# nubcico/EAV

Measured on AMD Instinct MI355X. Metric: EEGNet training samples/sec (fwd+CE+bwd+Adam), whole job, higher is better.
Workload: dtype f32; 1 GPU; EEGNet_tor(5, Chans=30, Samples=10000, kernLength=300, F1=8, D=8, F2=64) train step on x[64,1,30,10000] fp32 per GPU (BASELINE.json configs[1]); global_batch=64, per_gpu_batch=64, parallelism=dp1

## Files before the change

### eav_amd/_lib.py

```python
from __future__ import annotations

import ctypes as C
import os

_HERE = os.path.dirname(os.path.abspath(__file__))
LIB_PATH = os.environ.get("EAV_LIB_PATH") or os.path.join(_HERE, "libeav_hip.so")


class EavError(RuntimeError):
    pass


_p = C.c_void_p
_i = C.c_int
_i64 = C.c_int64
_u64 = C.c_uint64
_f = C.c_float
_d = C.c_double

SIGNATURES = {
    "eav_reduce_partials": [_p, _i, _i64, _i, _f, _p, _p],
    "eav_bn_finalize": [_p, _i, _i, _d, _p, _p, _p, _p, _i, _f, _f, _p, _p, _p, _p, _p],
    "eav_bn_bwd_finalize": [_p, _i, _i, _d, _i, _p, _p, _p, _p, _p],
    "eav_reduce_and_bn_bwd_finalize": [_p, _i, _i64, _i, _p, _p, _i, _i, _d, _i, _p, _p, _p, _p, _p, _i, _i, _d, _i, _p, _p, _p,
                                       _p, _p],
    "eav_renorm_rows": [_p, _i, _i, _f, _p],
    "eav_renorm_rows2": [_p, _i, _i, _p, _i, _i, _f, _p],
    "eav_eegnet_step_prologue": [_p, _p, _p, _p, _p, _p, _p, _p],
    "eav_eegnet_fir_fwd": [_p, _p, _p, _p, _i, _i, _i, _i, _p],
    "eav_eegnet_fir_wgrad": [_p, _p, _p, _p, _p, _i, _i, _i, _i, _p],
    "eav_eegnet_fir_fwd_indexed": [_p, _p, _p, _p, _p, _i, _i, _i, _i, _p],
    "eav_eegnet_fir_fwd_fft": [_p, _p, _p, _p, _p, _i, _i, _i, _i, _p],
    "eav_eegnet_fir_wgrad_fft": [_p, _p, _p, _p, _p, _p, _p, _i, _i, _i, _i, _p],
    "eav_eegnet_fir_wgrad_indexed": [_p, _p, _p, _p, _p, _p, _i, _i, _i, _i, _p],
    "eav_eegnet_dw_fwd": [_p, _p, _p, _p, _p, _i, _i, _i, _p],
    "eav_eegnet_dw_fwd_pool_eval": [_p, _p, _p, _p, _p, _p, _p, _i, _i, _i, _p],
    "eav_eegnet_dw_bwd": [_p, _p, _p, _p, _p, _p, _p, _i, _i, _i, _p],
    "eav_eegnet_dw_bwd_fused": [_p, _p, _p, _p, _p, _p, _p, _p, _p, _i, _i, _i, _f, _u64, _p, _p, _p],
    "eav_eegnet_dw_bwd_fused_eval": [_p, _p, _p, _p, _p, _p, _p, _p, _p, _p, _i, _i, _i, _f, _u64, _p, _p, _p],
    "eav_bn_elu_pool_fwd": [_p, _p, _p, _i, _i, _i, _i, _f, _u64, _p, _p, _p],
    "eav_bn_elu_pool_bwd_reduce": [_p, _p, _p, _p, _i, _i, _i, _i, _f, _u64, _p, _p, _p],
    "eav_bn_elu_pool_bwd_apply": [_p, _p, _p, _p, _p, _i, _i, _i, _i, _f, _u64, _p, _p, _p],
    "eav_bn_elu_pool_bwd_eval": [_p, _p, _p, _p, _p, _i, _i, _i, _i, _f, _u64, _p, _p, _p],
    "eav_conv64_prep_weights": [_p, _p, _p, _p],
    "eav_conv64_fwd": [_p, _p, _p, _p, _i, _i, _i, _p],
    "eav_conv64_wgrad": [_p, _p, _p, _i, _i, _i, _p],
    "eav_conv64_fft_fwd": [_p, _p, _p, _p, _p, _i, _i, _i, _p],
    "eav_conv64_fft_wgrad": [_p, _p, _p, _i, _i, _p],
    "eav_conv64_fft_bwd": [_p, _p, _p, _p, _p, _f, _u64, _p, _p, _p, _p, _p, _i, _i, _p],
    "eav_dense_softmax_fwd": [_p, _p, _p, _p, _p, _i, _i, _i, _p],
    "eav_dense_softmax_bwd": [_p, _p, _p, _p, _p, _p, _p, _i, _i, _i, _p],
    "eav_ce_fwd_bwd": [_p, _p, _p, _p, _p, _p, _i, _i, _p],
    "eav_dense_wide_fwd": [_p, _p, _p, _p, _i, _i, _i, _p],
    "eav_dense_wide_bwd": [_p, _p, _p, _p, _p, _p, _p, _i, _i, _i, _p],
    "eav_ce_wide_fwd_bwd": [_p, _p, _p, _p, _p, _p, _p, _i, _i, _p],
    "eav_bce_logits_fwd_bwd": [_p, _p, _p, _p, _p, _p, _i, _i, _p],
    "eav_mse_fwd_bwd": [_p, _p, _p, _p, _p, _i, _i, _p],
    "eav_scale_by_scalar": [_p, _p, _i64, _p],
    "eav_adam_step": [_p, _p, _p, _p, _i64, _f, _f, _f, _f, _f, _i64, _i, _p, _p],
    "eav_adam_step_scaled": [_p, _p, _p, _p, _i64, _f, _f, _f, _f, _f, _i64, _i, _p, _p, _p],
    "eav_grad_sumsq": [_p, _i, _i64, _p, _p],
    "eav_grad_fold": [_p, _p, _i, _i64, _p, _i, _p, _p],
    "eav_grad_clip_finish": [_p, _i64, _f, _p, _p],
    "eav_scale_ranges": [_p, _i, _i64, _p, _p],
    "eav_counter_inc": [_p, _p],
    "eav_counter_inc4": [_p, _p, _p, _p, _p],
# ... 245 lines not shown
```

### eav_amd/csrc/eav_common.hip

```cpp
#include "eav_common.h"

#include <stdarg.h>
#include <stdio.h>

#include "../../include/eav_hip.h"

static thread_local char g_err[512] = "";

int eav_set_error(int code, const char* fmt, ...) {
  va_list ap;
  va_start(ap, fmt);
  vsnprintf(g_err, sizeof(g_err), fmt, ap);
  va_end(ap);
  return code;
}

extern "C" const char* eav_last_error(void) { return g_err; }
extern "C" int eav_abi_version(void) { return EAV_ABI_VERSION; }

__global__ __launch_bounds__(256) void reduce_partials_kernel(const float* __restrict__ part, int nparts,
                                                              int64_t stride, int n, float scale,
                                                              float* __restrict__ out) {
  __shared__ double sh[16][17];
  const int ol = threadIdx.x & 15, pl = threadIdx.x >> 4;
// ... 129 lines not shown

extern "C" int eav_bn_finalize(const float* part, int nparts, int nch, double count, const float* gamma,
                               const float* beta, float* running_mean, float* running_var, int training,
                               float momentum, float eps, float* mean, float* invstd, float* scale, float* shift,
                               void* stream) {
  EAV_REQUIRE(nch > 0 && gamma && beta && running_mean && running_var && mean && invstd && scale && shift,
              "eav_bn_finalize: bad arguments");
  EAV_REQUIRE(!training || (part && nparts > 0 && count > 0), "eav_bn_finalize: training needs partials");
  hipLaunchKernelGGL(bn_finalize_kernel, dim3(nch), dim3(256), 0, (hipStream_t)stream, part, nparts, nch,
                     count, gamma, beta, running_mean, running_var, training, momentum, eps, mean, invstd, scale,
                     shift);
  EAV_CHECK_LAUNCH("eav_bn_finalize");
  return EAV_OK;
}

__device__ __forceinline__ void bn_bwd_finalize_body(const float* __restrict__ part, int nparts, int nch, double count,
                                                     int training, float* __restrict__ dgamma, float* __restrict__ dbeta,
                                                     float* __restrict__ m1, float* __restrict__ m2, int c) {
  __shared__ double shs[256], shq[256];
  double s = 0.0, q = 0.0;
  for (int p = threadIdx.x; p < nparts; p += 256) {
    s += (double)part[(int64_t)p * 2 * nch + c];
    q += (double)part[(int64_t)p * 2 * nch + nch + c];
  }
  shs[threadIdx.x] = s;
  shq[threadIdx.x] = q;
  __syncthreads();
  for (int o = 128; o > 0; o >>= 1) {
    if (threadIdx.x < o) {
      shs[threadIdx.x] += shs[threadIdx.x + o];
      shq[threadIdx.x] += shq[threadIdx.x + o];
    }
    __syncthreads();
  }
  if (threadIdx.x != 0) return;
  s = shs[0];
  q = shq[0];
  dbeta[c] = (float)s;
  dgamma[c] = (float)q;
  m1[c] = training ? (float)(s / count) : 0.f;
  m2[c] = training ? (float)(q / count) : 0.f;
}

__global__ void bn_bwd_finalize_kernel(const float* __restrict__ part, int nparts, int nch, double count,
                                       int training, float* __restrict__ dgamma, float* __restrict__ dbeta,
                                       float* __restrict__ m1, float* __restrict__ m2) {
  bn_bwd_finalize_body(part, nparts, nch, count, training, dgamma, dbeta, m1, m2, blockIdx.x);
}

struct BnBwdJob {
  const float* part;
  int nparts, nch, training;
  double count;
  float *dgamma, *dbeta, *m1, *m2;
};

// ... 36 lines not shown
                     n / 4, 1.f, out, nred, a, b);
  EAV_CHECK_LAUNCH("eav_reduce_and_bn_bwd_finalize");
  return EAV_OK;
}

extern "C" int eav_bn_bwd_finalize(const float* part, int nparts, int nch, double count, int training,
                                   float* dgamma, float* dbeta, float* m1, float* m2, void* stream) {
  EAV_REQUIRE(part && nparts > 0 && nch > 0 && count > 0 && dgamma && dbeta && m1 && m2,
              "eav_bn_bwd_finalize: bad arguments");
  hipLaunchKernelGGL(bn_bwd_finalize_kernel, dim3(nch), dim3(256), 0, (hipStream_t)stream, part, nparts,
                     nch, count, training, dgamma, dbeta, m1, m2);
  EAV_CHECK_LAUNCH("eav_bn_bwd_finalize");
  return EAV_OK;
}

__global__ void renorm_rows_kernel(float* __restrict__ w, int rows, int cols, float maxnorm, float* __restrict__ w_b,
                                   int cols_b) {
  __shared__ float red[8];
  int r = blockIdx.x;
  if (r >= rows) {
    r -= rows;
    w = w_b;
    cols = cols_b;
  }
  float* row = w + (int64_t)r * cols;
  const bool vec = (cols & 3) == 0 && (reinterpret_cast<uintptr_t>(row) & 15) == 0;
  float v[1] = {0.f};
  if (vec) {
    const float4* row4 = reinterpret_cast<const float4*>(row);
    const int n4 = cols >> 2;
// ... 54 lines not shown
```

### eav_amd/csrc/eegnet_block.hip

```cpp
#include "eav_common.h"
#include "../../include/eav_hip.h"

namespace {

constexpr int F1 = 8, DD = 8, CHMAX = 32;

__device__ __forceinline__ void ld4s(const float* p, int i, int n, bool vec, float (&v)[4]) {
  if (vec && i + 3 < n) {
    const f32x4 a = __builtin_nontemporal_load(reinterpret_cast<const f32x4*>(p + i));
    v[0] = a[0]; v[1] = a[1]; v[2] = a[2]; v[3] = a[3];
  } else {
#pragma unroll
    for (int e = 0; e < 4; ++e) v[e] = (i + e < n) ? p[i + e] : 0.f;
  }
}
__device__ __forceinline__ void st4s(float* p, int i, int n, bool vec, const float (&v)[4]) {
  if (vec && i + 3 < n) {
    __builtin_nontemporal_store((f32x4){v[0], v[1], v[2], v[3]}, reinterpret_cast<f32x4*>(p + i));
  } else {
#pragma unroll
    for (int e = 0; e < 4; ++e)
      if (i + e < n) p[i + e] = v[e];
  }
}
// ... 96 lines not shown
      float ps = 0.f;
#pragma unroll
      for (int e = 0; e < 4; ++e) ps += elu_f(sc2 * acc[d][e] + sh2);
      p2[((int64_t)b * CH + ch) * (S / 4) + t / 4] = ps * 0.25f;
    }
  }
  block_sum_nt<NT, 16>(st, red);
  if (threadIdx.x < 16) {
    const int nch = F1 * DD;
    float* dst = part + ((int64_t)b * gridDim.x + chunk) * 2 * nch;
    const int d = threadIdx.x & 7;
    dst[(threadIdx.x < 8 ? 0 : nch) + f * DD + d] = st[0];
  }
}

template <int P>
__global__ __launch_bounds__(256) void pool_fwd_kernel(const float* __restrict__ in, const float* __restrict__ bn,
                                                       float* __restrict__ out, int CH, int T, float drop_p,
                                                       uint64_t seed_in,
    const uint8_t* __restrict__ mask, const uint64_t* __restrict__ seed_dev) {
  const uint64_t seed = dropout_seed(seed_in, seed_dev);
  const int row = blockIdx.x, ch = row % CH;
  const float sc = bn[2 * CH + ch], sh = bn[3 * CH + ch];
  const int To = T / P;
  const float* src = in + (int64_t)row * T;
  const bool vec = (T & 3) == 0;
  for (int to = threadIdx.x; to < To; to += 256) {
    float s = 0.f;
#pragma unroll
    for (int j = 0; j < P; j += 4) {
      float v[4];
      ld4(src, to * P + j, T, vec, v);
#pragma unroll
      for (int e = 0; e < 4; ++e) s += elu_f(sc * v[e] + sh);
    }
    const uint64_t oi = (uint64_t)row * To + to;
    out[oi] = s * (1.0f / P) * dropout_mult_row(drop_p, seed, mask, oi, (uint64_t)row);
  }
}

template <int P>
__global__ __launch_bounds__(256) void pool_bwd_reduce_kernel(const float* __restrict__ dp,
                                                              const float* __restrict__ u,
                                                              const float* __restrict__ bn, float* __restrict__ part,
                                                              int CH, int T, float drop_p, uint64_t seed_in,
    const uint8_t* __restrict__ mask, const uint64_t* __restrict__ seed_dev) {
  const uint64_t seed = dropout_seed(seed_in, seed_dev);
  __shared__ float red[8];
  const int row = blockIdx.x, ch = row % CH, b = row / CH;
  const float mean = bn[ch], invstd = bn[CH + ch], sc = bn[2 * CH + ch], sh = bn[3 * CH + ch];
  const int To = T / P;
  const float* src = u + (int64_t)row * T;
// ... 311 lines not shown
                                       int B, int C, int S, float drop_p, uint64_t seed, const uint8_t* mask,
                                       const uint64_t* seed_dev, void* stream) {
  return dw_bwd_fused_launch("eav_eegnet_dw_bwd_fused", y1, z, dp2, bn2, bn1, w2, g1, stat_part, w_part, nullptr, B, C, S,
                             drop_p, seed, mask, seed_dev, stream);
}

extern "C" int eav_eegnet_dw_bwd_fused_eval(const float* y1, const float* z, const float* dp2, const float* bn2,
                                            const float* bn1, const float* w2, float* g1, float* stat_part, float* w_part,
                                            float* bn2_part, int B, int C, int S, float drop_p, uint64_t seed,
                                            const uint8_t* mask, const uint64_t* seed_dev, void* stream) {
  EAV_REQUIRE(bn2_part, "eav_eegnet_dw_bwd_fused_eval: bad arguments");
  return dw_bwd_fused_launch("eav_eegnet_dw_bwd_fused_eval", y1, z, dp2, bn2, bn1, w2, g1, stat_part, w_part, bn2_part, B, C,
                             S, drop_p, seed, mask, seed_dev, stream);
}

extern "C" int eav_bn_elu_pool_fwd(const float* in, const float* bn, float* out, int B, int CH, int T, int P,
                                   float drop_p, uint64_t seed, const uint8_t* mask, const uint64_t* seed_dev, void* stream) {
  EAV_REQUIRE(in && bn && out && B > 0 && CH > 0 && T >= P, "eav_bn_elu_pool_fwd: bad arguments");
  EAV_REQUIRE(P == 4 || P == 8, "eav_bn_elu_pool_fwd: pool %d not in {4,8}", P);
  EAV_REQUIRE(drop_p > -1.f && drop_p < 1.f, "eav_bn_elu_pool_fwd: dropout %f outside (-1,1)", drop_p);
  if (P == 4)
    hipLaunchKernelGGL(pool_fwd_kernel<4>, dim3(B * CH), dim3(256), 0, (hipStream_t)stream, in, bn, out, CH, T,
                       drop_p, seed, mask, seed_dev);
  else
    hipLaunchKernelGGL(pool_fwd_kernel<8>, dim3(B * CH), dim3(256), 0, (hipStream_t)stream, in, bn, out, CH, T,
                       drop_p, seed, mask, seed_dev);
  EAV_CHECK_LAUNCH("eav_bn_elu_pool_fwd");
  return EAV_OK;
}

extern "C" int eav_bn_elu_pool_bwd_reduce(const float* dp, const float* u, const float* bn, float* part, int B,
                                          int CH, int T, int P, float drop_p, uint64_t seed, const uint8_t* mask,
                                          const uint64_t* seed_dev, void* stream) {
  EAV_REQUIRE(dp && u && bn && part && B > 0 && CH > 0 && T >= P, "eav_bn_elu_pool_bwd_reduce: bad arguments");
  EAV_REQUIRE(P == 4 || P == 8, "eav_bn_elu_pool_bwd_reduce: pool %d not in {4,8}", P);
  if (P == 4)
    hipLaunchKernelGGL(pool_bwd_reduce_kernel<4>, dim3(B * CH), dim3(256), 0, (hipStream_t)stream, dp, u, bn, part,
                       CH, T, drop_p, seed, mask, seed_dev);
  else
    hipLaunchKernelGGL(pool_bwd_reduce_kernel<8>, dim3(B * CH), dim3(256), 0, (hipStream_t)stream, dp, u, bn, part,
                       CH, T, drop_p, seed, mask, seed_dev);
  EAV_CHECK_LAUNCH("eav_bn_elu_pool_bwd_reduce");
  return EAV_OK;
// ... 33 lines not shown
```

### eav_amd/csrc/head_optim.hip

```cpp
#include "eav_common.h"
#include "../../include/eav_hip.h"

namespace {

constexpr int NCMAX = 16;

__global__ __launch_bounds__(1024) void dense_softmax_fwd_kernel(const float* __restrict__ in,
                                                                 const float* __restrict__ w,
                                                                 const float* __restrict__ bias,
                                                                 float* __restrict__ logits, float* __restrict__ probs,
                                                                 int NF, int NC) {
  __shared__ float red[16 * NCMAX];
  const int b = blockIdx.x;
  const int lane = threadIdx.x & 63, wave = threadIdx.x >> 6;
  const float* src = in + (int64_t)b * NF;
  float acc[NCMAX];
#pragma unroll
  for (int j = 0; j < NCMAX; ++j) acc[j] = 0.f;
  if ((NF & 3) == 0) {
    const int nq = NF >> 2;
    if (NC <= 5) {
      for (int i0 = threadIdx.x; i0 < nq; i0 += 4096) {
        float4 v[4], wv[4][5];
#pragma unroll
// ... 45 lines not shown
    lg[threadIdx.x] = s + bias[threadIdx.x];
  }
  __syncthreads();
  if (threadIdx.x == 0) {
    float mx = lg[0];
    for (int j = 1; j < NC; ++j) mx = fmaxf(mx, lg[j]);
    float e[NCMAX], s = 0.f;
    for (int j = 0; j < NC; ++j) { e[j] = expf(lg[j] - mx); s += e[j]; }
    for (int j = 0; j < NC; ++j) {
      if (logits) logits[b * NC + j] = lg[j];
      if (probs) probs[b * NC + j] = e[j] / s;
    }
  }
}

__global__ __launch_bounds__(256) void dense_softmax_bwd_kernel(const float* __restrict__ dout,
                                                                const float* __restrict__ probs,
                                                                const float* __restrict__ in,
                                                                const float* __restrict__ w, float* __restrict__ dw,
                                                                float* __restrict__ dbias, float* __restrict__ din,
                                                                int B, int NF, int NC) {
  extern __shared__ float dl[];
  float* pw = dl + B * NC;
  for (int idx = threadIdx.x; idx < B * NC; idx += blockDim.x) {
    const int b = idx / NC;
    float v = dout[idx];
    if (probs) {
      float dot = 0.f;
      for (int j = 0; j < NC; ++j) dot += dout[b * NC + j] * probs[b * NC + j];
      v = probs[idx] * (v - dot);
    }
    dl[idx] = v;
  }
  __syncthreads();
  if (blockIdx.x == 0 && threadIdx.x < NC) {
    float s = 0.f;
    for (int b = 0; b < B; ++b) s += dl[b * NC + threadIdx.x];
    dbias[threadIdx.x] = s;
  }
  const int f = threadIdx.x & 63, slice = threadIdx.x >> 6;
  const int i = blockIdx.x * 64 + f;
  const bool live = i < NF;
  float wv[NCMAX], acc[NCMAX];
#pragma unroll
  for (int j = 0; j < NCMAX; ++j) {
    wv[j] = (live && j < NC) ? w[(int64_t)j * NF + i] : 0.f;
    acc[j] = 0.f;
  }
  for (int b0 = slice; b0 < B; b0 += 32) {
    float v[8];
#pragma unroll
    for (int u = 0; u < 8; ++u) v[u] = (live && b0 + 4 * u < B) ? in[(int64_t)(b0 + 4 * u) * NF + i] : 0.f;
#pragma unroll
    for (int u = 0; u < 8; ++u) {
      const int b = b0 + 4 * u;
      if (b < B) {
        float d = 0.f;
#pragma unroll
        for (int j = 0; j < NCMAX; ++j)
          if (j < NC) {
            const float g = dl[b * NC + j];
            acc[j] += g * v[u];
            d += wv[j] * g;
          }
        if (din && live) din[(int64_t)b * NF + i] = d;
      }
    }
  }
#pragma unroll
  for (int j = 0; j < NCMAX; ++j) pw[(slice * NCMAX + j) * 64 + f] = acc[j];
  __syncthreads();
  if (slice == 0 && live) {
#pragma unroll
    for (int j = 0; j < NCMAX; ++j)
      if (j < NC)
        dw[(int64_t)j * NF + i] = (pw[j * 64 + f] + pw[(NCMAX + j) * 64 + f]) + (pw[(2 * NCMAX + j) * 64 + f] + pw[(3 * NCMAX + j) * 64 + f]);
  }
}

__global__ __launch_bounds__(256) void ce_kernel(const float* __restrict__ in, const int64_t* __restrict__ y,
                                                 float* __restrict__ loss, float* __restrict__ din,
                                                 int* __restrict__ ncorrect, int* __restrict__ bad_label, int B,
                                                 int NC) {
  __shared__ float red[12];
  float nv[1] = {0.f};
  for (int b = threadIdx.x; b < B; b += 256) {
// ... 68 lines not shown
extern "C" int eav_dense_softmax_fwd(const float* in, const float* w, const float* bias, float* logits, float* probs,
                                     int B, int NF, int NC, void* stream) {
  EAV_REQUIRE(in && w && bias && (logits || probs) && B > 0 && NF > 0 && NC > 0 && NC <= NCMAX,
              "eav_dense_softmax_fwd: bad arguments (classes <= %d)", NCMAX);
  hipLaunchKernelGGL(dense_softmax_fwd_kernel, dim3(B), dim3(1024), 0, (hipStream_t)stream, in, w, bias, logits, probs,
                     NF, NC);
  EAV_CHECK_LAUNCH("eav_dense_softmax_fwd");
  return EAV_OK;
}

extern "C" int eav_dense_softmax_bwd(const float* dout, const float* probs, const float* in, const float* w,
                                     float* dw, float* dbias, float* din, int B, int NF, int NC, void* stream) {
  EAV_REQUIRE(dout && in && w && dw && dbias && B > 0 && NF > 0 && NC > 0 && NC <= NCMAX,
              "eav_dense_softmax_bwd: bad arguments (classes <= %d)", NCMAX);
  EAV_REQUIRE((size_t)B * NC * sizeof(float) <= 40 * 1024, "eav_dense_softmax_bwd: batch %d too large", B);
  hipLaunchKernelGGL(dense_softmax_bwd_kernel, dim3(cdiv(NF, 64)), dim3(256),
                     (B * NC + 4 * NCMAX * 64) * sizeof(float), (hipStream_t)stream, dout, probs, in, w, dw, dbias, din, B,
                     NF, NC);
  EAV_CHECK_LAUNCH("eav_dense_softmax_bwd");
  return EAV_OK;
}

extern "C" int eav_ce_fwd_bwd(const float* in, const int64_t* y, float* loss, float* din, int* ncorrect,
                              int* bad_label, int B, int NC, void* stream) {
  EAV_REQUIRE(in && y && B > 0 && NC > 0, "eav_ce_fwd_bwd: bad arguments");
  hipLaunchKernelGGL(ce_kernel, dim3(1), dim3(256), 0, (hipStream_t)stream, in, y, loss, din, ncorrect, bad_label, B,
                     NC);
  EAV_CHECK_LAUNCH("eav_ce_fwd_bwd");
  return EAV_OK;
}

__global__ __launch_bounds__(256) void scale_by_scalar_kernel(float* __restrict__ v, const float* __restrict__ sc,
                                                              int64_t n) {
  const float s = *sc;
// ... 130 lines not shown
```

### eav_amd/eegnet.py

```python
from __future__ import annotations

import os

import torch
import torch.nn as nn

from . import _lib
from .eegnet_paths import _PARAM_ORDER, FastPath, GenericPath, IndexedBatch
from .optim import CrossEntropyLoss, FusedAdam
from .runtime import (DeviceLoader, GraphStep, KernelFn, KernelModule, cached_workspace, eager_step,
                      gather_batch, train_step)


class _EEGNetFn(KernelFn):
    @staticmethod
    def forward(ctx, x, model, *params):
        out = KernelFn.forward(ctx, x, model, *params)
        ctx.probs_version = model._saved.probs._version
        return out

    @staticmethod
    def backward(ctx, dprobs):
        saved = ctx.model._saved
        if saved is not None and saved.token == ctx.token and saved.probs._version != ctx.probs_version:
# ... 25 lines not shown
        self.separableBN = nn.BatchNorm2d(F2)
        self.separablePool = nn.AvgPool2d((1, 8))
        self.flatten = nn.Flatten()
        self.dense = nn.Linear(F2 * (Samples // 4 // 8), nb_classes)
        self.softmax = nn.Softmax(dim=1)

        self.nb_classes, self.Chans, self.Samples, self.kernLength = nb_classes, Chans, Samples, kernLength
        self.F1, self.D, self.F2 = F1, D, F2
        self.norm_rate, self.dropoutRate = float(norm_rate), float(dropoutRate)
        self.spatial_dropout = dropoutType != 'Dropout'
        self.dropout_seed = 0x0EA5EED
        self.apply_max_norm = True
        self.fir_algo = os.environ.get("EAV_FIR_ALGO", "auto")
        self.conv_algo = os.environ.get("EAV_CONV_ALGO", "auto")
        self.conv_fuse = os.environ.get("EAV_CONV_FUSE", "1") != "0"
        self._infer = False
        self.fused_eval = False

    def _use_fft(self):
        return self._path.use_fft()

    def _run(self, x):
        self._require_same_device(x)
        self._ensure_flat()
        self._infer = (not torch.is_grad_enabled()) and (not self.training)
        return _EEGNetFn.apply(x, self, *self._params())

    def forward(self, x):
        self._require_gpu(x)
        if x.dim() == 3:
# ... 95 lines not shown
```

### eav_amd/eegnet_paths.py

```python
from __future__ import annotations

from typing import NamedTuple, Optional

import torch

from . import _lib, eegnet_canon
from .eegnet_canon import Saved
from .runtime import BN_M1, BN_M2, bn_field

_PARAM_ORDER = [
    "firstConv.weight", "firstBN.weight", "firstBN.bias",
    "depthwiseConv.weight", "depthwiseBN.weight", "depthwiseBN.bias",
    "separableConv.weight", "separableBN.weight", "separableBN.bias",
    "dense.weight", "dense.bias",
]


class IndexedBatch:

    def __init__(self, data, idx, step_begin=None):
        self.data, self.idx = data, idx
        self.shape = (idx.numel(),) + tuple(data.shape[1:])
        self.device = data.device
        self.step_begin, self.merged = step_begin, False
# ... 55 lines not shown
        self.np_fir_fft = _lib.plain("eav_eegnet_fir_fwd_fft_nparts", B, C, S)
        self.part_fir = f(max(self.np_fir, self.np_fir_fft), 16)
        self.fft_ws = None
        self.part_dw = f(B * nchunk, 128)
        self.np_c3 = _lib.plain("eav_conv64_fwd_nparts", B, T2)
        self.np_c3_fft = _lib.plain("eav_conv64_fft_nparts", B, T2)
        self.part_c3 = f(max(self.np_c3, self.np_c3_fft), 128)
        self.c64_ws = None
        self.part_pb = f(B, 128)
        self.part_dst = f(B * nchunk, 16)
        self.part_dw2 = f(B * nchunk, 64 * C)
        self.np_fw = _lib.plain("eav_eegnet_fir_wgrad_nparts", B, C, S)
        self.part_fw = f(self.np_fw, 8 * klen)
        self.np_cw = _lib.plain("eav_conv64_wgrad_nparts", B, T2)
        self.part_cw = f(self.np_cw, 64 * 1024)


class FastPath(_Path):
    st = None

    def use_fft(self):
        m = self.m
        if m.fir_algo not in ("auto", "fft", "mfma"):
            raise ValueError(f"fir_algo {m.fir_algo!r}: expected 'auto', 'fft' or 'mfma'")
        if m.fir_algo == "mfma" or m.kernLength > _lib.plain("eav_eegnet_fir_fft_max_taps"):
            return False
        return m.fir_algo == "fft" or m.Samples >= 1408

    def use_conv_fft(self, B):
        m = self.m
        if m.conv_algo not in ("auto", "fft", "mfma"):
            raise ValueError(f"conv_algo {m.conv_algo!r}: expected 'auto', 'fft' or 'mfma'")
        if m.conv_algo == "mfma":
            return False
        return m.conv_algo == "fft" or B * (m.Samples // 4) >= 40000

    def step_begin_args(self, optimizer, ys, idx, targets):
        return (optimizer.device_step_counter().data_ptr(), ys.data_ptr(), idx.data_ptr(), targets.data_ptr(), idx.numel())

    def forward(self, x):
        m = self.m
        self.st = _lib.stream_ptr()
        xp, xidx, B = self.input_view(x)
        C, S = m.Chans, m.Samples
        ws = m._workspace((B, C, S, str(x.device)), lambda: _Workspace(B, C, S, m.kernLength, m.nb_classes, x.device))
        training = bool(m.training)
        m._token += 1
        cnt, drop1, drop2, mk = self.dropout_args(x.device, training)
        conv_fft = self.use_conv_fft(B)
        begin = x.step_begin if xidx is not None else None
        if self.begin_step(ws, cnt, training, conv_fft, begin):
            x.merged = True
        if m.fused_eval and m._infer and not training and S % 4 == 0:
            self.block1_infer(ws, xp, xidx, B)
        else:
            self.fir_forward(ws, xp, xidx, B, training)
            self.block1_tail_forward(ws, B, training, drop1)
        self.separable_forward(ws, B, training, conv_fft)
        probs = self.head_forward(ws, B, drop2, x.device)
        m._saved = Saved(m._token, x, training, drop1, drop2, mk, ws, probs)
        return m._token

    def begin_step(self, ws, cnt, training, conv_fft, begin):
        L, P, st = _lib.call, _lib.ptr, self.st
        counters = self.counters(cnt, training)
        if not conv_fft:
            L("eav_eegnet_step_prologue", P(self.m.separableConv.weight), P(ws.wTf), P(ws.wTb), *counters, st)
        elif begin is not None:
            L("eav_step_begin", *counters, *begin, st)
            return True
        elif cnt is not None or training:
            L("eav_counter_inc4", *counters, st)
        return False

# ... 35 lines not shown

    def separable_forward(self, ws, B, training, conv_fft):
        m, L, P, st = self.m, _lib.call, _lib.ptr, self.st
        if conv_fft:
            if ws.c64_ws is None:
                ws.c64_ws = torch.zeros(_lib.plain("eav_conv64_fft_ws_floats", B, ws.T2), dtype=torch.float32,
                                        device=ws.y1.device)
            np_c3 = ws.np_c3_fft
            L("eav_conv64_fft_fwd", P(ws.p2), P(m.separableConv.weight), P(ws.u3), P(ws.part_c3), P(ws.c64_ws), B, ws.T2, 0,
              st)
        else:
            np_c3 = ws.np_c3
            L("eav_conv64_fwd", P(ws.p2), P(ws.wTf), P(ws.u3), P(ws.part_c3), B, ws.T2, 7, st)
        m._bn_finalize(m.separableBN, ws.part_c3, np_c3, B * ws.T2, ws.bn3, training)

    def head_forward(self, ws, B, drop2, dev):
        m, L, P, st = self.m, _lib.call, _lib.ptr, self.st
        nb, wd = m.nb_classes, P(m.dense.weight)
        L("eav_bn_elu_pool_fwd", P(ws.u3), P(ws.bn3), P(ws.p3), B, 64, ws.T2, 8, *drop2, st)
        probs = torch.empty(B, nb, dtype=torch.float32, device=dev)
        L("eav_dense_softmax_fwd", P(ws.p3), wd, P(m.dense.bias), None, P(probs), B, ws.NF, nb, st)
        if m.apply_max_norm:
            L("eav_renorm_rows2", P(m.depthwiseConv.weight), 64, m.Chans, wd, nb, ws.NF, m.norm_rate, st)
        return probs

    def backward(self, dprobs):
        m, s = self.m, self.m._saved
        self.st = _lib.stream_ptr()
        xp, xidx, B = self.input_view(s.x)
        g = m._grad_views()
        conv_fft = self.use_conv_fft(B)
        fuse = bool(m.conv_fuse) and conv_fft
        self.head_backward(s, g, B, dprobs)
        self.block2_tail_backward(s, g, B, fuse)
        self.separable_backward(s, g, B, conv_fft, fuse)
        self.depthwise_backward(s, g, B)
        self.fir_wgrad(s, g, xp, xidx, B)
        return m._grads_out(g)

    def head_backward(self, s, g, B, dprobs):
        m, ws, P = self.m, s.ws, _lib.ptr
        _lib.call("eav_dense_softmax_bwd", P(dprobs), P(s.probs), P(ws.p3), P(m.dense.weight), P(g["dense.weight"]),
                  P(g["dense.bias"]), P(ws.dp3), B, ws.NF, m.nb_classes, self.st)

    def block2_tail_backward(self, s, g, B, fuse):
        m, ws, L, P, st = self.m, s.ws, _lib.call, _lib.ptr, self.st
        gw, gb = g["separableBN.weight"], g["separableBN.bias"]
        if s.training:
            m._bn_elu_pool_bwd(ws.dp3, ws.u3, None if fuse else ws.du3, ws.bn3, ws.part_pb, gw, gb, B, 64, ws.T2, 8, s.drop2,
                               s.training)
        else:
            L("eav_bn_elu_pool_bwd_eval", P(ws.dp3), P(ws.u3), P(ws.bn3), P(ws.du3), P(ws.part_pb), B, 64, ws.T2, 8,
              *s.drop2, st)
            L("eav_bn_bwd_finalize", P(ws.part_pb), B, 64, float(B * ws.T2), int(s.training), P(gw), P(gb),
              bn_field(ws.bn3, 64, BN_M1), bn_field(ws.bn3, 64, BN_M2), st)

    def separable_backward(self, s, g, B, conv_fft, fuse):
        m, ws, L, P, st = self.m, s.ws, _lib.call, _lib.ptr, self.st
        T2, gw3 = ws.T2, P(g["separableConv.weight"])
        if fuse:
            L("eav_conv64_fft_bwd", None if s.training else P(ws.du3), P(ws.dp3), P(ws.u3), P(ws.bn3),
              bn_field(ws.bn3, 64, BN_M1), *s.drop2, P(ws.dp2), gw3, P(ws.c64_ws), B, T2, st)
        elif conv_fft:
# ... 108 lines not shown
```

### include/eav_hip.h

```cpp
#ifndef EAV_HIP_H
#define EAV_HIP_H
#include <stdint.h>

#ifdef __cplusplus
extern "C" {
#endif

#define EAV_ABI_VERSION 3

const char* eav_last_error(void);
int eav_abi_version(void);

int eav_reduce_partials(const float* part, int nparts, int64_t stride, int n, float scale, float* out, void* stream);

int eav_bn_finalize(const float* part, int nparts, int nch, double count, const float* gamma, const float* beta,
                    float* running_mean, float* running_var, int training, float momentum, float eps, float* mean,
                    float* invstd, float* scale, float* shift, void* stream);
int eav_bn_bwd_finalize(const float* part, int nparts, int nch, double count, int training, float* dgamma,
                        float* dbeta, float* m1, float* m2, void* stream);
int eav_reduce_and_bn_bwd_finalize(const float* part, int nparts, int64_t stride, int n, float* out,
                                   const float* part_a, int nparts_a, int nch_a, double count_a, int training_a,
                                   float* dgamma_a, float* dbeta_a, float* m1_a, float* m2_a,
                                   const float* part_b, int nparts_b, int nch_b, double count_b, int training_b,
                                   float* dgamma_b, float* dbeta_b, float* m1_b, float* m2_b, void* stream);
int eav_renorm_rows(float* w, int rows, int cols, float maxnorm, void* stream);
int eav_renorm_rows2(float* w_a, int rows_a, int cols_a, float* w_b, int rows_b, int cols_b, float maxnorm,
                     void* stream);

int eav_eegnet_fir_fwd_nparts(int B, int C, int S);
int eav_eegnet_fir_fwd(const float* x, const float* w1, float* y1, float* stat_part, int B, int C, int S, int klen,
                       void* stream);
int eav_eegnet_block1_infer(const float* x, const int64_t* xidx, const float* w1, const float* bn1, const float* w2,
                            const float* bn2, float* p2, int B, int C, int S, int klen, void* stream);
int eav_eegnet_fir_wgrad_nparts(int B, int C, int S);
// ... 16 lines not shown
                                const float* bn2, float* p2, int B, int C, int S, void* stream);
int eav_eegnet_dw_bwd(const float* y1, const float* dz, const float* bn1, const float* w2, float* g1,
                      float* stat_part, float* w_part, int B, int C, int S, void* stream);

int eav_eegnet_dw_bwd_fused(const float* y1, const float* z, const float* dp2, const float* bn2, const float* bn1,
                            const float* w2, float* g1, float* stat_part, float* w_part, int B, int C, int S,
                            float drop_p, uint64_t seed, const uint8_t* mask, const uint64_t* seed_dev, void* stream);

int eav_eegnet_dw_bwd_fused_eval(const float* y1, const float* z, const float* dp2, const float* bn2, const float* bn1,
                                 const float* w2, float* g1, float* stat_part, float* w_part, float* bn2_part, int B, int C,
                                 int S, float drop_p, uint64_t seed, const uint8_t* mask, const uint64_t* seed_dev,
                                 void* stream);

int eav_bn_elu_pool_fwd(const float* in, const float* bn, float* out, int B, int CH, int T, int P, float drop_p,
                        uint64_t seed, const uint8_t* mask, const uint64_t* seed_dev, void* stream);
int eav_bn_elu_pool_bwd_reduce(const float* dp, const float* u, const float* bn, float* part , int B,
                               int CH, int T, int P, float drop_p, uint64_t seed, const uint8_t* mask,
                               const uint64_t* seed_dev, void* stream);
int eav_bn_elu_pool_bwd_apply(const float* dp, const float* u, const float* bn, const float* m12 ,
                              float* du, int B, int CH, int T, int P, float drop_p, uint64_t seed,
                              const uint8_t* mask, const uint64_t* seed_dev, void* stream);
int eav_bn_elu_pool_bwd_eval(const float* dp, const float* u, const float* bn, float* du, float* part , int B,
                             int CH, int T, int P, float drop_p, uint64_t seed, const uint8_t* mask,
                             const uint64_t* seed_dev, void* stream);

int eav_conv64_prep_weights(const float* w , float* wT_fwd , float* wT_bwd, void* stream);
int eav_eegnet_step_prologue(const float* w, float* wT_fwd, float* wT_bwd, int64_t* c0, int64_t* c1, int64_t* c2,
                             int64_t* c3, void* stream);
int eav_conv64_ntiles(int T);
int eav_conv64_fwd_nparts(int B, int T);
// ... 26 lines not shown
                  int K, int transposed, void* stream);
int eav_dconv_wgrad(const float* dy, const float* x, float* part, int B, int Cin, int Cout, int T, int K, void* stream);
int eav_sepconv_fwd_nparts(int B, int T);
int eav_sepconv_fwd(const float* a, const float* wdw, const float* wp, float* d3, float* z, float* stat_part, int B,
                    int C2, int F2, int T, int K2, void* stream);
int eav_pointwise_bwd_nparts(int B, int T);
int eav_pointwise_bwd(const float* du, const float* d3, const float* wp, float* dd3, float* w_part, int B, int C2,
                      int F2, int T, void* stream);
int eav_dwt_bwd(const float* dd3, const float* a, const float* wdw, float* da, float* w_part, int B, int C2, int T,
                int K2, void* stream);

int eav_dense_softmax_fwd(const float* in, const float* w, const float* bias, float* logits, float* probs, int B,
                          int NF, int NC, void* stream);
int eav_dense_softmax_bwd(const float* dout, const float* probs, const float* in, const float* w, float* dw,
                          float* dbias, float* din, int B, int NF, int NC, void* stream);
int eav_ce_fwd_bwd(const float* in, const int64_t* y, float* loss, float* din, int* ncorrect, int* bad_label, int B,
                   int NC, void* stream);
#define EAV_HEAD_MAX_CLASSES 32768
int eav_dense_wide_fwd(const float* in, const float* w, const float* bias, float* logits, int B, int NF, int NC,
                       void* stream);
int64_t eav_dense_wide_bwd_ws_floats(int B, int NF, int NC);
int eav_dense_wide_bwd(const float* dlogits, const float* in, const float* w, float* dw, float* dbias, float* din,
                       float* ws, int B, int NF, int NC, void* stream);
int64_t eav_ce_wide_ws_floats(int B);
int eav_ce_wide_fwd_bwd(const float* in, const int64_t* y, float* loss, float* din, int* ncorrect, int* bad_label,
                        float* ws, int B, int NC, void* stream);
int64_t eav_head_loss_ws_floats(int B);
int eav_bce_logits_fwd_bwd(const float* logits, const float* targets, float* loss, float* dlogits, int* nhits, float* ws,
                           int B, int NC, void* stream);
int eav_mse_fwd_bwd(const float* logits, const float* targets, float* loss, float* dlogits, float* ws, int B, int NC,
// ... 250 lines not shown
```

Measured before the change: 48010 samples/s.

## Precompute pooled BN-backward side products in forward to skip reduce pass

The BN+ELU+avgpool forward now also writes per-pooled-output sums of the ELU gradient and of the ELU gradient times the normalized input, scaled by the pool and dropout factor. The dense head backward dots these with the pooled gradient to produce per-feature BN backward sums, and a new finalize kernel reduces them per channel. This removes the separate full-resolution bwd_reduce pass over the T2-length activations, at the cost of two extra pooled-size buffers written in forward and read in backward. It is enabled by default through EAV_BN_SUMS=pooled.

Result: no change. 48300 samples/s, median of 6 (+0.6%).

```diff
diff --git a/eav_amd/_lib.py b/eav_amd/_lib.py
--- a/eav_amd/_lib.py
+++ b/eav_amd/_lib.py
@@ -22,6 +22,7 @@
     "eav_reduce_partials": [_p, _i, _i64, _i, _f, _p, _p],
     "eav_bn_finalize": [_p, _i, _i, _d, _p, _p, _p, _p, _i, _f, _f, _p, _p, _p, _p, _p],
     "eav_bn_bwd_finalize": [_p, _i, _i, _d, _i, _p, _p, _p, _p, _p],
+    "eav_bn_bwd_finalize_feat": [_p, _i, _i, _d, _i, _p, _p, _p, _p, _p],
     "eav_reduce_and_bn_bwd_finalize": [_p, _i, _i64, _i, _p, _p, _i, _i, _d, _i, _p, _p, _p, _p, _p, _i, _i, _d, _i, _p, _p, _p,
                                        _p, _p],
     "eav_renorm_rows": [_p, _i, _i, _f, _p],
@@ -39,6 +40,7 @@
     "eav_eegnet_dw_bwd_fused": [_p, _p, _p, _p, _p, _p, _p, _p, _p, _i, _i, _i, _f, _u64, _p, _p, _p],
     "eav_eegnet_dw_bwd_fused_eval": [_p, _p, _p, _p, _p, _p, _p, _p, _p, _p, _i, _i, _i, _f, _u64, _p, _p, _p],
     "eav_bn_elu_pool_fwd": [_p, _p, _p, _i, _i, _i, _i, _f, _u64, _p, _p, _p],
+    "eav_bn_elu_pool_fwd_q": [_p, _p, _p, _p, _p, _i, _i, _i, _i, _f, _u64, _p, _p, _p],
     "eav_bn_elu_pool_bwd_reduce": [_p, _p, _p, _p, _i, _i, _i, _i, _f, _u64, _p, _p, _p],
     "eav_bn_elu_pool_bwd_apply": [_p, _p, _p, _p, _p, _i, _i, _i, _i, _f, _u64, _p, _p, _p],
     "eav_bn_elu_pool_bwd_eval": [_p, _p, _p, _p, _p, _i, _i, _i, _i, _f, _u64, _p, _p, _p],
@@ -50,6 +52,7 @@
     "eav_conv64_fft_bwd": [_p, _p, _p, _p, _p, _f, _u64, _p, _p, _p, _p, _p, _i, _i, _p],
     "eav_dense_softmax_fwd": [_p, _p, _p, _p, _p, _i, _i, _i, _p],
     "eav_dense_softmax_bwd": [_p, _p, _p, _p, _p, _p, _p, _i, _i, _i, _p],
+    "eav_dense_softmax_bwd_q": [_p, _p, _p, _p, _p, _p, _p, _p, _p, _p, _i, _i, _i, _p],
     "eav_ce_fwd_bwd": [_p, _p, _p, _p, _p, _p, _i, _i, _p],
     "eav_dense_wide_fwd": [_p, _p, _p, _p, _i, _i, _i, _p],
     "eav_dense_wide_bwd": [_p, _p, _p, _p, _p, _p, _p, _i, _i, _i, _p],
diff --git a/eav_amd/csrc/eav_common.hip b/eav_amd/csrc/eav_common.hip
--- a/eav_amd/csrc/eav_common.hip
+++ b/eav_amd/csrc/eav_common.hip
@@ -167,14 +167,15 @@
   return EAV_OK;
 }
 
-__device__ __forceinline__ void bn_bwd_finalize_body(const float* __restrict__ part, int nparts, int nch, double count,
-                                                     int training, float* __restrict__ dgamma, float* __restrict__ dbeta,
-                                                     float* __restrict__ m1, float* __restrict__ m2, int c) {
+__device__ __forceinline__ void bn_bwd_finalize_terms(const float* __restrict__ ps, const float* __restrict__ pq,
+                                                      int64_t stride, int nparts, double count, int training,
+                                                      float* __restrict__ dgamma, float* __restrict__ dbeta,
+                                                      float* __restrict__ m1, float* __restrict__ m2, int c) {
   __shared__ double shs[256], shq[256];
   double s = 0.0, q = 0.0;
   for (int p = threadIdx.x; p < nparts; p += 256) {
-    s += (double)part[(int64_t)p * 2 * nch + c];
-    q += (double)part[(int64_t)p * 2 * nch + nch + c];
+    s += (double)ps[p * stride];
+    q += (double)pq[p * stride];
   }
   shs[threadIdx.x] = s;
   shq[threadIdx.x] = q;
@@ -193,6 +194,19 @@
   dgamma[c] = (float)q;
   m1[c] = training ? (float)(s / count) : 0.f;
   m2[c] = training ? (float)(q / count) : 0.f;
+}
+
+__device__ __forceinline__ void bn_bwd_finalize_body(const float* __restrict__ part, int nparts, int nch, double count,
+                                                     int training, float* __restrict__ dgamma, float* __restrict__ dbeta,
+                                                     float* __restrict__ m1, float* __restrict__ m2, int c) {
+  bn_bwd_finalize_terms(part + c, part + nch + c, 2 * (int64_t)nch, nparts, count, training, dgamma, dbeta, m1, m2, c);
+}
+
+__global__ void bn_bwd_finalize_feat_kernel(const float* __restrict__ fs, int NF, int nch, double count, int training,
+                                            float* __restrict__ dgamma, float* __restrict__ dbeta, float* __restrict__ m1,
+                                            float* __restrict__ m2) {
+  const int c = blockIdx.x, per = NF / nch;
+  bn_bwd_finalize_terms(fs + (int64_t)c * per, fs + NF + (int64_t)c * per, 1, per, count, training, dgamma, dbeta, m1, m2, c);
 }
 
 __global__ void bn_bwd_finalize_kernel(const float* __restrict__ part, int nparts, int nch, double count,
@@ -259,6 +273,16 @@
   return EAV_OK;
 }
 
+extern "C" int eav_bn_bwd_finalize_feat(const float* fs, int NF, int nch, double count, int training, float* dgamma,
+                                        float* dbeta, float* m1, float* m2, void* stream) {
+  EAV_REQUIRE(fs && nch > 0 && NF >= nch && NF % nch == 0 && count > 0 && dgamma && dbeta && m1 && m2,
+              "eav_bn_bwd_finalize_feat: bad arguments (NF a multiple of nch)");
+  hipLaunchKernelGGL(bn_bwd_finalize_feat_kernel, dim3(nch), dim3(256), 0, (hipStream_t)stream, fs, NF, nch, count,
+                     training, dgamma, dbeta, m1, m2);
+  EAV_CHECK_LAUNCH("eav_bn_bwd_finalize_feat");
+  return EAV_OK;
+}
+
 __global__ void renorm_rows_kernel(float* __restrict__ w, int rows, int cols, float maxnorm, float* __restrict__ w_b,
                                    int cols_b) {
   __shared__ float red[8];
diff --git a/eav_amd/csrc/eegnet_block.hip b/eav_amd/csrc/eegnet_block.hip
--- a/eav_amd/csrc/eegnet_block.hip
+++ b/eav_amd/csrc/eegnet_block.hip
@@ -134,28 +134,45 @@
   }
 }
 
-template <int P>
+template <int P, bool SIDE>
 __global__ __launch_bounds__(256) void pool_fwd_kernel(const float* __restrict__ in, const float* __restrict__ bn,
                                                        float* __restrict__ out, int CH, int T, float drop_p,
                                                        uint64_t seed_in,
-    const uint8_t* __restrict__ mask, const uint64_t* __restrict__ seed_dev) {
+    const uint8_t* __restrict__ mask, const uint64_t* __restrict__ seed_dev, float* __restrict__ q1,
+                                                       float* __restrict__ q2) {
   const uint64_t seed = dropout_seed(seed_in, seed_dev);
   const int row = blockIdx.x, ch = row % CH;
   const float sc = bn[2 * CH + ch], sh = bn[3 * CH + ch];
+  const float mean = SIDE ? bn[ch] : 0.f, invstd = SIDE ? bn[CH + ch] : 0.f;
   const int To = T / P;
   const float* src = in + (int64_t)row * T;
   const bool vec = (T & 3) == 0;
   for (int to = threadIdx.x; to < To; to += 256) {
-    float s = 0.f;
+    float s = 0.f, e1 = 0.f, e2 = 0.f;
 #pragma unroll
     for (int j = 0; j < P; j += 4) {
       float v[4];
       ld4(src, to * P + j, T, vec, v);
 #pragma unroll
-      for (int e = 0; e < 4; ++e) s += elu_f(sc * v[e] + sh);
+      for (int e = 0; e < 4; ++e) {
+        const float pre = sc * v[e] + sh;
+        const float a = elu_f(pre);
+        s += a;
+        if constexpr (SIDE) {
+          const float eg = elu_grad_from_out(pre, a);
+          e1 += eg;
+          e2 += eg * ((v[e] - mean) * invstd);
+        }
+      }
     }
     const uint64_t oi = (uint64_t)row * To + to;
-    out[oi] = s * (1.0f / P) * dropout_mult_row(drop_p, seed, mask, oi, (uint64_t)row);
+    const float dm = dropout_mult_row(drop_p, seed, mask, oi, (uint64_t)row);
+    out[oi] = s * (1.0f / P) * dm;
+    if constexpr (SIDE) {
+      const float k = (1.0f / P) * dm;
+      q1[oi] = k * e1;
+      q2[oi] = k * e2;
+    }
   }
 }
 
@@ -497,19 +514,36 @@
                              S, drop_p, seed, mask, seed_dev, stream);
 }
 
+static int pool_fwd_launch(const char* name, const float* in, const float* bn, float* out, float* q1, float* q2, int B, int CH,
+                           int T, int P, float drop_p, uint64_t seed, const uint8_t* mask, const uint64_t* seed_dev,
+                           void* stream) {
+  EAV_REQUIRE(in && bn && out && B > 0 && CH > 0 && T >= P, "%s: bad arguments", name);
+  EAV_REQUIRE(P == 4 || P == 8, "%s: pool %d not in {4,8}", name, P);
+  EAV_REQUIRE(drop_p > -1.f && drop_p < 1.f, "%s: dropout %f outside (-1,1)", name, drop_p);
+#define POOL_FWD_LAUNCH(PP, SIDE)                                                                                        \
+  hipLaunchKernelGGL((pool_fwd_kernel<PP, SIDE>), dim3(B * CH), dim3(256), 0, (hipStream_t)stream, in, bn, out, CH, T, \
+                     drop_p, seed, mask, seed_dev, q1, q2)
+  if (q1) {
+    if (P == 4) POOL_FWD_LAUNCH(4, true); else POOL_FWD_LAUNCH(8, true);
+  } else {
+    if (P == 4) POOL_FWD_LAUNCH(4, false); else POOL_FWD_LAUNCH(8, false);
+  }
+#undef POOL_FWD_LAUNCH
+  EAV_CHECK_LAUNCH(name);
+  return EAV_OK;
+}
+
 extern "C" int eav_bn_elu_pool_fwd(const float* in, const float* bn, float* out, int B, int CH, int T, int P,
                                    float drop_p, uint64_t seed, const uint8_t* mask, const uint64_t* seed_dev, void* stream) {
-  EAV_REQUIRE(in && bn && out && B > 0 && CH > 0 && T >= P, "eav_bn_elu_pool_fwd: bad arguments");
-  EAV_REQUIRE(P == 4 || P == 8, "eav_bn_elu_pool_fwd: pool %d not in {4,8}", P);
-  EAV_REQUIRE(drop_p > -1.f && drop_p < 1.f, "eav_bn_elu_pool_fwd: dropout %f outside (-1,1)", drop_p);
-  if (P == 4)
-    hipLaunchKernelGGL(pool_fwd_kernel<4>, dim3(B * CH), dim3(256), 0, (hipStream_t)stream, in, bn, out, CH, T,
-                       drop_p, seed, mask, seed_dev);
-  else
-    hipLaunchKernelGGL(pool_fwd_kernel<8>, dim3(B * CH), dim3(256), 0, (hipStream_t)stream, in, bn, out, CH, T,
-                       drop_p, seed, mask, seed_dev);
-  EAV_CHECK_LAUNCH("eav_bn_elu_pool_fwd");
-  return EAV_OK;
+  return pool_fwd_launch("eav_bn_elu_pool_fwd", in, bn, out, nullptr, nullptr, B, CH, T, P, drop_p, seed, mask, seed_dev,
+                         stream);
+}
+
+extern "C" int eav_bn_elu_pool_fwd_q(const float* in, const float* bn, float* out, float* q1, float* q2, int B, int CH,
+                                     int T, int P, float drop_p, uint64_t seed, const uint8_t* mask,
+                                     const uint64_t* seed_dev, void* stream) {
+  EAV_REQUIRE(q1 && q2, "eav_bn_elu_pool_fwd_q: bad arguments");
+  return pool_fwd_launch("eav_bn_elu_pool_fwd_q", in, bn, out, q1, q2, B, CH, T, P, drop_p, seed, mask, seed_dev, stream);
 }
 
 extern "C" int eav_bn_elu_pool_bwd_reduce(const float* dp, const float* u, const float* bn, float* part, int B,
diff --git a/eav_amd/csrc/head_optim.hip b/eav_amd/csrc/head_optim.hip
--- a/eav_amd/csrc/head_optim.hip
+++ b/eav_amd/csrc/head_optim.hip
@@ -83,12 +83,14 @@
   }
 }
 
+template <bool SIDE>
 __global__ __launch_bounds__(256) void dense_softmax_bwd_kernel(const float* __restrict__ dout,
                                                                 const float* __restrict__ probs,
                                                                 const float* __restrict__ in,
                                                                 const float* __restrict__ w, float* __restrict__ dw,
                                                                 float* __restrict__ dbias, float* __restrict__ din,
-                                                                int B, int NF, int NC) {
+                                                                int B, int NF, int NC, const float* __restrict__ q1,
+                                                                const float* __restrict__ q2, float* __restrict__ fs) {
   extern __shared__ float dl[];
   float* pw = dl + B * NC;
   for (int idx = threadIdx.x; idx < B * NC; idx += blockDim.x) {
@@ -116,10 +118,18 @@
     wv[j] = (live && j < NC) ? w[(int64_t)j * NF + i] : 0.f;
     acc[j] = 0.f;
   }
+  float sq[2] = {0.f, 0.f};
   for (int b0 = slice; b0 < B; b0 += 32) {
-    float v[8];
-#pragma unroll
-    for (int u = 0; u < 8; ++u) v[u] = (live && b0 + 4 * u < B) ? in[(int64_t)(b0 + 4 * u) * NF + i] : 0.f;
+    float v[8], qa[8], qb[8];
+#pragma unroll
+    for (int u = 0; u < 8; ++u) {
+      const bool ok = live && b0 + 4 * u < B;
+      v[u] = ok ? in[(int64_t)(b0 + 4 * u) * NF + i] : 0.f;
+      if constexpr (SIDE) {
+        qa[u] = ok ? q1[(int64_t)(b0 + 4 * u) * NF + i] : 0.f;
+        qb[u] = ok ? q2[(int64_t)(b0 + 4 * u) * NF + i] : 0.f;
+      }
+    }
 #pragma unroll
     for (int u = 0; u < 8; ++u) {
       const int b = b0 + 4 * u;
@@ -133,12 +143,29 @@
             d += wv[j] * g;
           }
         if (din && live) din[(int64_t)b * NF + i] = d;
+        if constexpr (SIDE) {
+          sq[0] += d * qa[u];
+          sq[1] += d * qb[u];
+        }
       }
     }
   }
 #pragma unroll
   for (int j = 0; j < NCMAX; ++j) pw[(slice * NCMAX + j) * 64 + f] = acc[j];
+  if constexpr (SIDE) {
+    float* ps = pw + 4 * NCMAX * 64;
+    ps[(slice * 2 + 0) * 64 + f] = sq[0];
+    ps[(slice * 2 + 1) * 64 + f] = sq[1];
+  }
   __syncthreads();
+  if constexpr (SIDE) {
+    const float* ps = pw + 4 * NCMAX * 64;
+    if (slice == 1 && live) {
+#pragma unroll
+      for (int k = 0; k < 2; ++k)
+        fs[(int64_t)k * NF + i] = (ps[k * 64 + f] + ps[(2 + k) * 64 + f]) + (ps[(4 + k) * 64 + f] + ps[(6 + k) * 64 + f]);
+    }
+  }
   if (slice == 0 && live) {
 #pragma unroll
     for (int j = 0; j < NCMAX; ++j)
@@ -237,10 +264,23 @@
   EAV_REQUIRE(dout && in && w && dw && dbias && B > 0 && NF > 0 && NC > 0 && NC <= NCMAX,
               "eav_dense_softmax_bwd: bad arguments (classes <= %d)", NCMAX);
   EAV_REQUIRE((size_t)B * NC * sizeof(float) <= 40 * 1024, "eav_dense_softmax_bwd: batch %d too large", B);
-  hipLaunchKernelGGL(dense_softmax_bwd_kernel, dim3(cdiv(NF, 64)), dim3(256),
+  hipLaunchKernelGGL(dense_softmax_bwd_kernel<false>, dim3(cdiv(NF, 64)), dim3(256),
                      (B * NC + 4 * NCMAX * 64) * sizeof(float), (hipStream_t)stream, dout, probs, in, w, dw, dbias, din, B,
-                     NF, NC);
+                     NF, NC, nullptr, nullptr, nullptr);
   EAV_CHECK_LAUNCH("eav_dense_softmax_bwd");
+  return EAV_OK;
+}
+
+extern "C" int eav_dense_softmax_bwd_q(const float* dout, const float* probs, const float* in, const float* w, float* dw,
+                                       float* dbias, float* din, const float* q1, const float* q2, float* fs, int B, int NF,
+                                       int NC, void* stream) {
+  EAV_REQUIRE(dout && in && w && dw && dbias && din && q1 && q2 && fs && B > 0 && NF > 0 && NC > 0 && NC <= NCMAX,
+              "eav_dense_softmax_bwd_q: bad arguments (classes <= %d)", NCMAX);
+  EAV_REQUIRE((size_t)B * NC * sizeof(float) <= 40 * 1024, "eav_dense_softmax_bwd_q: batch %d too large", B);
+  hipLaunchKernelGGL(dense_softmax_bwd_kernel<true>, dim3(cdiv(NF, 64)), dim3(256),
+                     (B * NC + 4 * NCMAX * 64 + 4 * 2 * 64) * sizeof(float), (hipStream_t)stream, dout, probs, in, w, dw,
+                     dbias, din, B, NF, NC, q1, q2, fs);
+  EAV_CHECK_LAUNCH("eav_dense_softmax_bwd_q");
   return EAV_OK;
 }
 
diff --git a/eav_amd/eegnet.py b/eav_amd/eegnet.py
--- a/eav_amd/eegnet.py
+++ b/eav_amd/eegnet.py
@@ -63,6 +63,7 @@
         self.fir_algo = os.environ.get("EAV_FIR_ALGO", "auto")
         self.conv_algo = os.environ.get("EAV_CONV_ALGO", "auto")
         self.conv_fuse = os.environ.get("EAV_CONV_FUSE", "1") != "0"
+        self.bn_sums = os.environ.get("EAV_BN_SUMS", "pooled")
         self._infer = False
         self.fused_eval = False
 
diff --git a/eav_amd/eegnet_paths.py b/eav_amd/eegnet_paths.py
--- a/eav_amd/eegnet_paths.py
+++ b/eav_amd/eegnet_paths.py
@@ -93,6 +93,14 @@
         self.part_fw = f(self.np_fw, 8 * klen)
         self.np_cw = _lib.plain("eav_conv64_wgrad_nparts", B, T2)
         self.part_cw = f(self.np_cw, 64 * 1024)
+        self.q1_8 = self.q2_8 = self.fs = None
+        self.q_token = None
+
+    def side_products(self, B):
+        if self.fs is None:
+            f = lambda *shape: torch.empty(*shape, dtype=torch.float32, device=self.y1.device)
+            self.q1_8, self.q2_8 = f(B, 64, self.T3), f(B, 64, self.T3)
+            self.fs = f(2, self.NF)
 
 
 class FastPath(_Path):
@@ -113,6 +121,12 @@
         if m.conv_algo == "mfma":
             return False
         return m.conv_algo == "fft" or B * (m.Samples // 4) >= 40000
+
+    def use_pooled_sums(self):
+        m = self.m
+        if m.bn_sums not in ("pooled", "passes"):
+            raise ValueError(f"bn_sums {m.bn_sums!r}: expected 'pooled' or 'passes'")
+        return m.bn_sums == "pooled"
 
     def step_begin_args(self, optimizer, ys, idx, targets):
         return (optimizer.device_step_counter().data_ptr(), ys.data_ptr(), idx.data_ptr(), targets.data_ptr(), idx.numel())
@@ -127,6 +141,10 @@
         m._token += 1
         cnt, drop1, drop2, mk = self.dropout_args(x.device, training)
         conv_fft = self.use_conv_fft(B)
+        pooled = self.use_pooled_sums() and training
+        if pooled:
+            ws.side_products(B)
+        ws.q_token = m._token if pooled else None
         begin = x.step_begin if xidx is not None else None
         if self.begin_step(ws, cnt, training, conv_fft, begin):
             x.merged = True
@@ -136,7 +154,7 @@
             self.fir_forward(ws, xp, xidx, B, training)
             self.block1_tail_forward(ws, B, training, drop1)
         self.separable_forward(ws, B, training, conv_fft)
-        probs = self.head_forward(ws, B, drop2, x.device)
+        probs = self.head_forward(ws, B, drop2, x.device, pooled)
         m._saved = Saved(m._token, x, training, drop1, drop2, mk, ws, probs)
         return m._token
 
@@ -202,10 +220,13 @@
             L("eav_conv64_fwd", P(ws.p2), P(ws.wTf), P(ws.u3), P(ws.part_c3), B, ws.T2, 7, st)
         m._bn_finalize(m.separableBN, ws.part_c3, np_c3, B * ws.T2, ws.bn3, training)
 
-    def head_forward(self, ws, B, drop2, dev):
+    def head_forward(self, ws, B, drop2, dev, pooled):
         m, L, P, st = self.m, _lib.call, _lib.ptr, self.st
         nb, wd = m.nb_classes, P(m.dense.weight)
-        L("eav_bn_elu_pool_fwd", P(ws.u3), P(ws.bn3), P(ws.p3), B, 64, ws.T2, 8, *drop2, st)
+        if pooled:
+            L("eav_bn_elu_pool_fwd_q", P(ws.u3), P(ws.bn3), P(ws.p3), P(ws.q1_8), P(ws.q2_8), B, 64, ws.T2, 8, *drop2, st)
+        else:
+            L("eav_bn_elu_pool_fwd", P(ws.u3), P(ws.bn3), P(ws.p3), B, 64, ws.T2, 8, *drop2, st)
         probs = torch.empty(B, nb, dtype=torch.float32, device=dev)
         L("eav_dense_softmax_fwd", P(ws.p3), wd, P(m.dense.bias), None, P(probs), B, ws.NF, nb, st)
         if m.apply_max_norm:
@@ -219,22 +240,31 @@
         g = m._grad_views()
         conv_fft = self.use_conv_fft(B)
         fuse = bool(m.conv_fuse) and conv_fft
-        self.head_backward(s, g, B, dprobs)
-        self.block2_tail_backward(s, g, B, fuse)
+        pooled = s.training and s.ws.q_token == s.token
+        self.head_backward(s, g, B, dprobs, pooled)
+        self.block2_tail_backward(s, g, B, fuse, pooled)
         self.separable_backward(s, g, B, conv_fft, fuse)
         self.depthwise_backward(s, g, B)
         self.fir_wgrad(s, g, xp, xidx, B)
         return m._grads_out(g)
 
-    def head_backward(self, s, g, B, dprobs):
+    def head_backward(self, s, g, B, dprobs, pooled):
         m, ws, P = self.m, s.ws, _lib.ptr
-        _lib.call("eav_dense_softmax_bwd", P(dprobs), P(s.probs), P(ws.p3), P(m.dense.weight), P(g["dense.weight"]),
-                  P(g["dense.bias"]), P(ws.dp3), B, ws.NF, m.nb_classes, self.st)
-
-    def block2_tail_backward(self, s, g, B, fuse):
+        args = (P(dprobs), P(s.probs), P(ws.p3), P(m.dense.weight), P(g["dense.weight"]), P(g["dense.bias"]), P(ws.dp3))
+        if pooled:
+            _lib.call("eav_dense_softmax_bwd_q", *args, P(ws.q1_8), P(ws.q2_8), P(ws.fs), B, ws.NF, m.nb_classes, self.st)
+        else:
+            _lib.call("eav_dense_softmax_bwd", *args, B, ws.NF, m.nb_classes, self.st)
+
+    def block2_tail_backward(self, s, g, B, fuse, pooled):
         m, ws, L, P, st = self.m, s.ws, _lib.call, _lib.ptr, self.st
         gw, gb = g["separableBN.weight"], g["separableBN.bias"]
-        if s.training:
+        if pooled:
+            m1, m2 = bn_field(ws.bn3, 64, BN_M1), bn_field(ws.bn3, 64, BN_M2)
+            L("eav_bn_bwd_finalize_feat", P(ws.fs), ws.NF, 64, float(B * ws.T2), int(s.training), P(gw), P(gb), m1, m2, st)
+            if not fuse:
+                L("eav_bn_elu_pool_bwd_apply", P(ws.dp3), P(ws.u3), P(ws.bn3), m1, P(ws.du3), B, 64, ws.T2, 8, *s.drop2, st)
+        elif s.training:
             m._bn_elu_pool_bwd(ws.dp3, ws.u3, None if fuse else ws.du3, ws.bn3, ws.part_pb, gw, gb, B, 64, ws.T2, 8, s.drop2,
                                s.training)
         else:
diff --git a/include/eav_hip.h b/include/eav_hip.h
--- a/include/eav_hip.h
+++ b/include/eav_hip.h
@@ -18,6 +18,8 @@
                     float* invstd, float* scale, float* shift, void* stream);
 int eav_bn_bwd_finalize(const float* part, int nparts, int nch, double count, int training, float* dgamma,
                         float* dbeta, float* m1, float* m2, void* stream);
+int eav_bn_bwd_finalize_feat(const float* fs, int NF, int nch, double count, int training, float* dgamma, float* dbeta,
+                             float* m1, float* m2, void* stream);
 int eav_reduce_and_bn_bwd_finalize(const float* part, int nparts, int64_t stride, int n, float* out,
                                    const float* part_a, int nparts_a, int nch_a, double count_a, int training_a,
                                    float* dgamma_a, float* dbeta_a, float* m1_a, float* m2_a,
@@ -64,6 +66,8 @@
 
 int eav_bn_elu_pool_fwd(const float* in, const float* bn, float* out, int B, int CH, int T, int P, float drop_p,
                         uint64_t seed, const uint8_t* mask, const uint64_t* seed_dev, void* stream);
+int eav_bn_elu_pool_fwd_q(const float* in, const float* bn, float* out, float* q1, float* q2, int B, int CH, int T, int P,
+                          float drop_p, uint64_t seed, const uint8_t* mask, const uint64_t* seed_dev, void* stream);
 int eav_bn_elu_pool_bwd_reduce(const float* dp, const float* u, const float* bn, float* part , int B,
                                int CH, int T, int P, float drop_p, uint64_t seed, const uint8_t* mask,
                                const uint64_t* seed_dev, void* stream);
@@ -120,6 +124,8 @@
                           int NF, int NC, void* stream);
 int eav_dense_softmax_bwd(const float* dout, const float* probs, const float* in, const float* w, float* dw,
                           float* dbias, float* din, int B, int NF, int NC, void* stream);
+int eav_dense_softmax_bwd_q(const float* dout, const float* probs, const float* in, const float* w, float* dw, float* dbias,
+                            float* din, const float* q1, const float* q2, float* fs, int B, int NF, int NC, void* stream);
 int eav_ce_fwd_bwd(const float* in, const int64_t* y, float* loss, float* din, int* ncorrect, int* bad_label, int B,
                    int NC, void* stream);
 #define EAV_HEAD_MAX_CLASSES 32768
```
